# mutiann/few-shot-transformer-tts

Measured on AMD Instinct MI355X. Metric: padded mel-frames/sec, full training step (fwd+loss+bwd+allreduce+Adam), higher is better.
Workload: dtype bf16; 1 GPU; LJSpeech-shaped (BASELINE configs[1]) packed batch per GPU: B=14 S=114 T=582, default hparams (83.5M params), dropout on, single speaker/language; global_batch=14, seq_len=582, parallelism=dp1

## Files before the change

### few-shot-transformer-tts_amd/csrc/attention32.hip

```cpp
#include "b2s_common.h"
#include "attention.h"

namespace {

typedef __attribute__((ext_vector_type(16))) float f32x16_t;
typedef __attribute__((ext_vector_type(4))) uint32_t u32x4_t;
typedef __attribute__((address_space(3))) bf16x4_t* lds_b64_ptr;

typedef __attribute__((address_space(1))) void* gptr_t;
typedef __attribute__((address_space(3))) void* lptr_t;
__device__ inline f32x16_t mma32(bf16x8_t a, bf16x8_t b, f32x16_t c) { return __builtin_amdgcn_mfma_f32_32x32x16_bf16(a, b, c, 0, 0, 0); }
__device__ inline float half_max(float v) {
    const uint32_t u = __float_as_uint(v);
    const auto r = __builtin_amdgcn_permlane32_swap(u, u, false, false);
    return fmaxf(__uint_as_float(r[0]), __uint_as_float(r[1]));
}
__device__ inline float half_sum(float v) {
    const uint32_t u = __float_as_uint(v);
    const auto r = __builtin_amdgcn_permlane32_swap(u, u, false, false);
    return __uint_as_float(r[0]) + __uint_as_float(r[1]);
}
__device__ inline float fast_exp2(float x) { return __builtin_amdgcn_exp2f(x); }
__device__ inline float vmax3(float a, float b, float c) { float d; asm("v_max3_f32 %0, %1, %2, %3" : "=v"(d) : "v"(a), "v"(b), "v"(c)); return d; }
constexpr float A32_LOG2E = 1.4426950408889634f, A32_LN2 = 0.6931471805599453f;
constexpr float A32_LAZY = 8.f;

template <int DH> __device__ inline int swz(int row) { return DH == 64 ? ((((row >> 1) & 1) << 2) | ((row >> 2) & 3)) : ((row >> 2) & 3); }

template <int DH, int NW> struct Dma {
    static constexpr int CPR = DH / 8, NI = CPR / NW;
    static_assert(CPR % NW == 0, "tile must split evenly over the waves");
    int row[NI], cb[NI];
    const char* base; uint32_t ldb; int last;
    __device__ inline void init(const bf16_t* b, long ld_, int nrows_, int wave, int lane) {
        base = reinterpret_cast<const char*>(b); ldb = (uint32_t)ld_ * 2u; last = nrows_ - 1;
#pragma unroll
        for (int i = 0; i < NI; ++i) {
            const int p = (wave * NI + i) * 64 + lane, r = p / CPR, c = (p - r * CPR) ^ swz<DH>(r);
            row[i] = r; cb[i] = c * 16;
        }
    }
    __device__ inline void issue(bf16_t* tile, int row0, int wave) const {
#pragma unroll
        for (int i = 0; i < NI; ++i) {
            const uint32_t voff = (uint32_t)min(row0 + row[i], last) * ldb + (uint32_t)cb[i];
            __builtin_amdgcn_global_load_lds((gptr_t)(base + voff), (lptr_t)(tile + (wave * NI + i) * 512), 16, 0, 0);
        }
    }
};
__device__ inline void cfence() { asm volatile("" ::: "memory"); }
__device__ inline void wait_vm0() { asm volatile("s_waitcnt vmcnt(0)" ::: "memory"); }
template <int DH> __device__ inline bf16x8_t frag_a(const bf16_t* tile, int row, int ks, int hi) {
    return *reinterpret_cast<const bf16x8_t*>(tile + row * DH + (((ks * 2 + hi) ^ swz<DH>(row)) * 8));
}
template <int DH> __device__ inline bf16x8_t frag_t(const bf16_t* tile, int rb, int d0, int lane) {
    const int li = lane & 15, g = lane >> 4;
    const int row = rb + (g >> 1) * 4 + (li >> 2), col = d0 + (g & 1) * 16 + (li & 3) * 4;
    const bf16_t* p0 = tile + row * DH + (((col >> 3) ^ swz<DH>(row)) * 8) + (col & 7);
    const bf16_t* p1 = tile + (row + 8) * DH + (((col >> 3) ^ swz<DH>(row + 8)) * 8) + (col & 7);
    const bf16x4_t lo = __builtin_amdgcn_ds_read_tr16_b64_v4i16((lds_b64_ptr)p0);
    const bf16x4_t hh = __builtin_amdgcn_ds_read_tr16_b64_v4i16((lds_b64_ptr)p1);
    bf16x8_t r;
    r[0] = lo[0]; r[1] = lo[1]; r[2] = lo[2]; r[3] = lo[3]; r[4] = hh[0]; r[5] = hh[1]; r[6] = hh[2]; r[7] = hh[3];
    return r;
}
template <int S8> __device__ inline bf16x8_t pack8(const f32x16_t& v) {
    const u32x4_t u = {f2bf2(v[S8 * 8 + 0], v[S8 * 8 + 1]), f2bf2(v[S8 * 8 + 2], v[S8 * 8 + 3]), f2bf2(v[S8 * 8 + 4], v[S8 * 8 + 5]),
                       f2bf2(v[S8 * 8 + 6], v[S8 * 8 + 7])};
    return __builtin_bit_cast(bf16x8_t, u);
}
__device__ inline bf16x8_t frag_own(const bf16_t* base, long ld, int row, int ks, int hi) {
    return *reinterpret_cast<const bf16x8_t*>(base + (long)row * ld + ks * 16 + hi * 8);
}
__device__ inline float frag_dot(bf16x8_t x, bf16x8_t y) {
    float s = 0.f;
#pragma unroll
    for (int e = 0; e < 8; ++e) s += bf2f((bf16_t)x[e]) * bf2f((bf16_t)y[e]);
    return s;
}
__device__ inline int crow(int r, int hi) { return (r & 3) + 8 * (r >> 2) + 4 * hi; }

__device__ inline void a32_block(int& rank, int& z) {
    const int nx = gridDim.x, Z = gridDim.y, orig = blockIdx.y * nx + blockIdx.x;
    if ((Z & 7) == 0) {
        const int zc = Z >> 3, x = orig & 7, i = orig >> 3;
        rank = i / zc; z = x * zc + (i - rank * zc);
    } else {
        const int nwg = nx * Z, xcd = orig & 7, q = nwg >> 3, r = nwg & 7;
        const int wg = (xcd < r ? xcd * (q + 1) : r * (q + 1) + (xcd - r) * q) + (orig >> 3);
        z = wg / nx; rank = wg - z * nx;
    }
}
template <int DH>
__device__ inline void store_own(bf16_t* dst, const f32x16_t (&acc)[DH / 32], float mul, int hi) {
#pragma unroll
    for (int dt = 0; dt < DH / 32; ++dt)
#pragma unroll
        for (int g4 = 0; g4 < 4; ++g4) {
            uint2 u;
            u.x = f2bf2(acc[dt][g4 * 4 + 0] * mul, acc[dt][g4 * 4 + 1] * mul);
            u.y = f2bf2(acc[dt][g4 * 4 + 2] * mul, acc[dt][g4 * 4 + 3] * mul);
            *reinterpret_cast<uint2*>(dst + dt * 32 + g4 * 8 + hi * 4) = u;
        }
}
template <int DH> __device__ inline void zero_own(bf16_t* dst, int hi) {
#pragma unroll
    for (int dt = 0; dt < DH / 32; ++dt)
#pragma unroll
        for (int g4 = 0; g4 < 4; ++g4) *reinterpret_cast<uint2*>(dst + dt * 32 + g4 * 8 + hi * 4) = make_uint2(0, 0);
}
constexpr uint32_t GOLD = 0x9E3779B1u;


template <int DH>
__device__ inline void first2(f32x16_t (&s)[2], const bf16_t* tile, const bf16x8_t (&own)[DH / 16], int l31, int hi) {
#pragma unroll
    for (int t = 0; t < 2; ++t) {
#pragma unroll
        for (int r = 0; r < 16; ++r) s[t][r] = 0.f;
#pragma unroll
        for (int ks = 0; ks < DH / 16; ++ks) s[t] = mma32(frag_a<DH>(tile, t * 32 + l31, ks, hi), own[ks], s[t]);
    }
}
template <int DH>
__device__ inline void first1(f32x16_t& s, const bf16_t* tile, int t, const bf16x8_t (&own)[DH / 16], int l31, int hi) {
#pragma unroll
    for (int r = 0; r < 16; ++r) s[r] = 0.f;
#pragma unroll
    for (int ks = 0; ks < DH / 16; ++ks) s = mma32(frag_a<DH>(tile, t * 32 + l31, ks, hi), own[ks], s);
}
template <int DH>
__device__ inline void second1(f32x16_t (&acc)[DH / 32], const bf16_t* tile, int t, const f32x16_t& w, int lane) {
    const bf16x8_t p0 = pack8<0>(w), p1 = pack8<1>(w);
#pragma unroll
    for (int dt = 0; dt < DH / 32; ++dt) {
        acc[dt] = mma32(frag_t<DH>(tile, t * 32, dt * 32, lane), p0, acc[dt]);
        acc[dt] = mma32(frag_t<DH>(tile, t * 32 + 16, dt * 32, lane), p1, acc[dt]);
    }
}
__device__ inline void quad_words(uint32_t (&wd)[16], uint32_t xrow, int k0) {
    const uint32_t xt = xrow + (uint32_t)(k0 >> 2) * GOLD;
#pragma unroll
    for (int t = 0; t < 2; ++t)
#pragma unroll
        for (int g4 = 0; g4 < 4; ++g4) {
            const uint32_t x = xt + (uint32_t)(t * 8 + g4 * 2) * GOLD, y = x ^ (x >> 16);
            wd[t * 8 + g4 * 2] = y * B2S_WC0; wd[t * 8 + g4 * 2 + 1] = y * B2S_WC1;
        }
}
__device__ inline uint32_t keep_mask16(uint32_t w, uint32_t tsm1, uint32_t fifteen) {
    uint32_t d, m;
    asm("v_pk_sub_i16 %0, %1, %2 clamp" : "=v"(d) : "v"(tsm1), "v"(w));
    asm("v_pk_ashrrev_i16 %0, %1, %2" : "=v"(m) : "v"(fifteen), "v"(d));
    return m;
}
template <int S8> __device__ inline bf16x8_t pack8_drop(const f32x16_t& v, const uint32_t* wd, uint32_t tsm1, uint32_t fifteen) {
    const u32x4_t u = {f2bf2(v[S8 * 8 + 0], v[S8 * 8 + 1]) & keep_mask16(wd[S8 * 4 + 0], tsm1, fifteen), f2bf2(v[S8 * 8 + 2], v[S8 * 8 + 3]) & keep_mask16(wd[S8 * 4 + 1], tsm1, fifteen),
                       f2bf2(v[S8 * 8 + 4], v[S8 * 8 + 5]) & keep_mask16(wd[S8 * 4 + 2], tsm1, fifteen), f2bf2(v[S8 * 8 + 6], v[S8 * 8 + 7]) & keep_mask16(wd[S8 * 4 + 3], tsm1, fifteen)};
    return __builtin_bit_cast(bf16x8_t, u);
}
template <int DH>
__device__ inline void second1p(f32x16_t (&acc)[DH / 32], const bf16_t* tile, int t, bf16x8_t p0, bf16x8_t p1, int lane) {
#pragma unroll
    for (int dt = 0; dt < DH / 32; ++dt) {
        acc[dt] = mma32(frag_t<DH>(tile, t * 32, dt * 32, lane), p0, acc[dt]);
        acc[dt] = mma32(frag_t<DH>(tile, t * 32 + 16, dt * 32, lane), p1, acc[dt]);
    }
}

template <int DH, int NW, bool DROP>
__global__ __launch_bounds__(NW * 64, 2) void attn32_fwd_kernel(AttnArgs a) {
    constexpr int NKS = DH / 16, NDT = DH / 32, TILE = 64 * DH, QB = NW * 32;
    __shared__ __attribute__((aligned(16))) bf16_t sK[2 * TILE];
    __shared__ __attribute__((aligned(16))) bf16_t sV[2 * TILE];
    const int tid = threadIdx.x, lane = tid & 63, wave = tid >> 6, l31 = lane & 31, hi = lane >> 5;
    int blk, z;
    a32_block(blk, z);
    blk = gridDim.x - 1 - blk;
    const int b = z / a.H, h = z - b * a.H;
    const int qrow0 = a.qoff ? a.qoff[b] : b * a.Lq, Lq = a.qoff ? a.qoff[b + 1] - qrow0 : a.Lq;
    const int krow0 = a.koff ? a.koff[b] : b * a.Lk, Lk = a.koff ? a.koff[b + 1] - krow0 : a.Lk;
    const int qb0 = blk * QB, qw0 = qb0 + wave * 32, q = qw0 + l31, qc = min(q, Lq - 1);
    const int qlive = a.qskip ? min(a.qskip[b], Lq) : Lq;
    const bool wlive = (qw0 & ~63) < qlive && qw0 < Lq;
    bf16_t* out = reinterpret_cast<bf16_t*>(a.out) + ((long)qrow0 + qc) * a.ldo + h * DH;
    if (!wlive && q < Lq) {
        zero_own<DH>(out, hi);
        if (hi == 0 && a.lse) a.lse[(long)z * a.Lq + q] = 0.f;
    }
    if (qb0 >= qlive) return;
    const bf16_t* Q = reinterpret_cast<const bf16_t*>(a.q) + (long)qrow0 * a.ldq + h * DH;
    const bf16_t* K = reinterpret_cast<const bf16_t*>(a.k) + (long)krow0 * a.ldk + h * DH;
    const bf16_t* V = reinterpret_cast<const bf16_t*>(a.v) + (long)krow0 * a.ldv + h * DH;
    const bool causal = a.mask_mode & 2;
    int kend = Lk;
    if (a.mask_mode & 1) kend = min(kend, a.klen[b]);
    int ktiles = (kend + 63) / 64;
    if (causal) {
        int qlast = min(qb0 + QB - 1, Lq - 1);
        if (a.qskip) qlast = min(qlast, ((qlive + 63) & ~63) - 1);
        ktiles = min(ktiles, qlast / 64 + 1);
    }
    const int wkt = !wlive ? 0 : (causal ? min(ktiles, min(qw0 + 31, Lq - 1) / 64 + 1) : ktiles);
    Dma<DH, NW> dmk, dmv;
    dmk.init(K, a.ldk, Lk, wave, lane); dmv.init(V, a.ldv, Lk, wave, lane);
    if (ktiles > 0) { dmk.issue(sK, 0, wave); dmv.issue(sV, 0, wave); }
    if (ktiles > 1) dmk.issue(sK + TILE, 64, wave);
    bf16x8_t qf[NKS];
#pragma unroll
    for (int ks = 0; ks < NKS; ++ks) qf[ks] = frag_own(Q, a.ldq, qc, ks, hi);

    f32x16_t o[NDT];
#pragma unroll
    for (int dt = 0; dt < NDT; ++dt)
#pragma unroll
        for (int r = 0; r < 16; ++r) o[dt][r] = 0.f;
    float m = -INFINITY, l = 0.f;
    const float sl2 = a.scale * A32_LOG2E;
    const uint32_t xrow = b2s_wseed(a.drop, (uint32_t)((long)z * a.Lq + qc)) + (uint32_t)hi * GOLD;
    const uint32_t tsm1 = ((uint32_t)(b2s_wthresh(a.drop) - 1) & 0xffffu) * 0x10001u, fifteen = 0x000f000fu;
    f32x16_t s0[2], s1[2];
    uint32_t wd[16];
    wait_vm0();
    __syncthreads();
    if (wkt > 0) {
        first2<DH>(s0, sK, qf, l31, hi);
        if (DROP) quad_words(wd, xrow, 0);
    }
    __syncthreads();
    auto iter = [&](const int kt, f32x16_t (&sc)[2], f32x16_t (&sn)[2]) {
        const int k0 = kt * 64, cur = kt & 1;
        if (kt + 2 < ktiles) dmk.issue(sK + cur * TILE, k0 + 128, wave);
        if (kt + 1 < ktiles) dmv.issue(sV + (cur ^ 1) * TILE, k0 + 64, wave);
        if (kt < wkt) {
            const bool interior = k0 + 64 <= kend && (!causal || k0 + 63 <= qw0);
            if (!interior) {
#pragma unroll
                for (int t = 0; t < 2; ++t)
#pragma unroll
                    for (int r = 0; r < 16; ++r) {
                        const int key = k0 + t * 32 + crow(r, hi);
                        sc[t][r] = (key < kend && (!causal || key <= q)) ? sc[t][r] : -INFINITY;
                    }
            }
            float mx = sc[0][0];
#pragma unroll
            for (int r = 0; r < 16; ++r) mx = vmax3(mx, sc[0][r], sc[1][r]);
            mx = half_max(mx) * sl2;
            const bool grow = mx > m + A32_LAZY;
            if (__any(grow)) {
                const float mn = grow ? mx : m;
                const float alpha = mn == m ? 1.f : fast_exp2(m - mn);
                m = mn; l *= alpha;
#pragma unroll
                for (int dt = 0; dt < NDT; ++dt)
#pragma unroll
                    for (int r = 0; r < 16; ++r) o[dt][r] *= alpha;
            }
            const float mref = m == -INFINITY ? 0.f : m;
            first2<DH>(sn, sK + (cur ^ 1) * TILE, qf, l31, hi);
#pragma unroll
            for (int t = 0; t < 2; ++t)
#pragma unroll
                for (int r = 0; r < 16; ++r) {
                    const float p = fast_exp2(fmaf(sc[t][r], sl2, -mref));
                    l += p;
                    sc[t][r] = p;
                }
            if (DROP) {
                second1p<DH>(o, sV + cur * TILE, 0, pack8_drop<0>(sc[0], wd, tsm1, fifteen), pack8_drop<1>(sc[0], wd, tsm1, fifteen), lane);
                second1p<DH>(o, sV + cur * TILE, 1, pack8_drop<0>(sc[1], wd + 8, tsm1, fifteen), pack8_drop<1>(sc[1], wd + 8, tsm1, fifteen), lane);
            } else {
                second1<DH>(o, sV + cur * TILE, 0, sc[0], lane);
                second1<DH>(o, sV + cur * TILE, 1, sc[1], lane);
            }
            if (DROP) quad_words(wd, xrow, k0 + 64);
        }
        wait_vm0();
        __syncthreads();
    };
    for (int kt = 0; kt < ktiles; kt += 2) {
        iter(kt, s0, s1);
        if (kt + 1 < ktiles) iter(kt + 1, s1, s0);
    }
    l = half_sum(l);
    if (wlive && q < Lq) {
        const float inv = 1.f / l;
        store_own<DH>(out, o, inv * a.drop.scale, hi);
        if (hi == 0 && a.lse) a.lse[(long)z * a.Lq + q] = (m + __log2f(l)) * A32_LN2;
    }
}

template <int DH, int NW, bool DROP>
__global__ __launch_bounds__(NW * 64, 2) void attn32_dq_kernel(AttnArgs a) {
    constexpr int NKS = DH / 16, NDT = DH / 32, TILE = 64 * DH, QB = NW * 32;
    __shared__ __attribute__((aligned(16))) bf16_t sK[2 * TILE];
    __shared__ __attribute__((aligned(16))) bf16_t sV[2 * TILE];
    const int tid = threadIdx.x, lane = tid & 63, wave = tid >> 6, l31 = lane & 31, hi = lane >> 5;
    int blk, z;
    a32_block(blk, z);
    blk = gridDim.x - 1 - blk;
    const int b = z / a.H, h = z - b * a.H;
    const int qrow0 = a.qoff ? a.qoff[b] : b * a.Lq, Lq = a.qoff ? a.qoff[b + 1] - qrow0 : a.Lq;
    const int krow0 = a.koff ? a.koff[b] : b * a.Lk, Lk = a.koff ? a.koff[b + 1] - krow0 : a.Lk;
    const int qb0 = blk * QB, qw0 = qb0 + wave * 32, q = qw0 + l31, qc = min(q, Lq - 1);
    const int qlive = a.qskip ? min(a.qskip[b], Lq) : Lq;
    const bool wlive = (qw0 & ~63) < qlive && qw0 < Lq;
    bf16_t* dqo = reinterpret_cast<bf16_t*>(a.dq) + ((long)qrow0 + qc) * a.lddq + h * DH;
    if (!wlive && q < Lq) {
        zero_own<DH>(dqo, hi);
        if (hi == 0) a.dsum[(long)z * a.Lq + q] = 0.f;
    }
    if (qb0 >= qlive) return;
    const bf16_t* Q = reinterpret_cast<const bf16_t*>(a.q) + (long)qrow0 * a.ldq + h * DH;
    const bf16_t* K = reinterpret_cast<const bf16_t*>(a.k) + (long)krow0 * a.ldk + h * DH;
    const bf16_t* V = reinterpret_cast<const bf16_t*>(a.v) + (long)krow0 * a.ldv + h * DH;
    const bf16_t* dO = reinterpret_cast<const bf16_t*>(a.dout) + (long)qrow0 * a.ldo + h * DH;
    const bf16_t* O = reinterpret_cast<const bf16_t*>(a.oref) + (long)qrow0 * a.ldo + h * DH;
    const bool causal = a.mask_mode & 2;
    int kend = Lk;
    if (a.mask_mode & 1) kend = min(kend, a.klen[b]);
    int ktiles = (kend + 63) / 64;
    if (causal) {
        int qlast = min(qb0 + QB - 1, Lq - 1);
        if (a.qskip) qlast = min(qlast, ((qlive + 63) & ~63) - 1);
        ktiles = min(ktiles, qlast / 64 + 1);
    }
    const int wkt = !wlive ? 0 : (causal ? min(ktiles, min(qw0 + 31, Lq - 1) / 64 + 1) : ktiles);
    Dma<DH, NW> dmk, dmv;
    dmk.init(K, a.ldk, Lk, wave, lane); dmv.init(V, a.ldv, Lk, wave, lane);
    if (ktiles > 0) { dmk.issue(sK, 0, wave); dmv.issue(sV, 0, wave); }
    bf16x8_t qf[NKS], dof[NKS];
    float Dq = 0.f;
#pragma unroll
    for (int ks = 0; ks < NKS; ++ks) {
        qf[ks] = frag_own(Q, a.ldq, qc, ks, hi); dof[ks] = frag_own(dO, a.ldo, qc, ks, hi);
        Dq += frag_dot(frag_own(O, a.ldo, qc, ks, hi), dof[ks]);
    }
    Dq = half_sum(Dq);
    if (wlive && hi == 0 && q < Lq) a.dsum[(long)z * a.Lq + q] = Dq;
    f32x16_t dq[NDT];
#pragma unroll
    for (int dt = 0; dt < NDT; ++dt)
#pragma unroll
        for (int r = 0; r < 16; ++r) dq[dt][r] = 0.f;
    const float sl2 = a.scale * A32_LOG2E, lse2 = a.lse[(long)z * a.Lq + qc] * A32_LOG2E;
    const uint32_t xrow = b2s_wseed(a.drop, (uint32_t)((long)z * a.Lq + qc)) + (uint32_t)hi * GOLD;
    const int ts32 = (int)((uint32_t)b2s_wthresh(a.drop) << 16);
    const float dscale = a.drop.scale;
    wait_vm0();
    __syncthreads();
    for (int kt = 0; kt < ktiles; ++kt) {
        const int k0 = kt * 64, cur = kt & 1;
        const bf16_t* tK = sK + cur * TILE;
        const bf16_t* tV = sV + cur * TILE;
        if (kt + 1 < ktiles) { dmk.issue(sK + (cur ^ 1) * TILE, k0 + 64, wave); dmv.issue(sV + (cur ^ 1) * TILE, k0 + 64, wave); }
        if (kt < wkt) {
            const bool interior = k0 + 64 <= kend && (!causal || k0 + 63 <= qw0);
            f32x16_t s[2], dp[2];
            first2<DH>(s, tK, qf, l31, hi);
            first2<DH>(dp, tV, dof, l31, hi);
            if (!interior) {
#pragma unroll
                for (int t = 0; t < 2; ++t)
#pragma unroll
                    for (int r = 0; r < 16; ++r) {
                        const int key = k0 + t * 32 + crow(r, hi);
                        s[t][r] = (key < kend && (!causal || key <= q)) ? s[t][r] : -INFINITY;
                    }
            }
            uint32_t wd[16];
            if (DROP) quad_words(wd, xrow, k0);
#pragma unroll
            for (int t = 0; t < 2; ++t) {
#pragma unroll
                for (int r = 0; r < 16; ++r) s[t][r] = fast_exp2(fmaf(s[t][r], sl2, -lse2));
                if (DROP) {
#pragma unroll
                    for (int pr = 0; pr < 8; ++pr) {
                        const uint32_t w = wd[t * 8 + pr];
                        dp[t][2 * pr] = (int)(w << 16) >= ts32 ? dp[t][2 * pr] * dscale : 0.f;
                        dp[t][2 * pr + 1] = (int)w >= ts32 ? dp[t][2 * pr + 1] * dscale : 0.f;
                    }
                }
#pragma unroll
                for (int r = 0; r < 16; ++r) s[t][r] = s[t][r] * (dp[t][r] - Dq);
                second1<DH>(dq, tK, t, s[t], lane);
            }
        }
        wait_vm0();
        __syncthreads();
    }
    if (wlive && q < Lq) store_own<DH>(dqo, dq, a.scale, hi);
}

template <int DH, int NW, bool DROP>
__global__ __launch_bounds__(NW * 64, 2) void attn32_dkv_kernel(AttnArgs a) {
    constexpr int NKS = DH / 16, NDT = DH / 32, TILE = 64 * DH, KB = NW * 32;
    __shared__ __attribute__((aligned(16))) bf16_t sQ[2 * TILE];
    __shared__ __attribute__((aligned(16))) bf16_t sO[2 * TILE];
    __shared__ __attribute__((aligned(16))) float sL[2 * 64], sD[2 * 64];
    __shared__ __attribute__((aligned(16))) uint32_t sS[2 * 64];
    const int tid = threadIdx.x, lane = tid & 63, wave = tid >> 6, l31 = lane & 31, hi = lane >> 5;
    int blk, z;
    a32_block(blk, z);
    const int b = z / a.H, h = z - b * a.H;
    const int qrow0 = a.qoff ? a.qoff[b] : b * a.Lq, Lq = a.qoff ? a.qoff[b + 1] - qrow0 : a.Lq;
    const int krow0 = a.koff ? a.koff[b] : b * a.Lk, Lk = a.koff ? a.koff[b + 1] - krow0 : a.Lk;
    const int kb0 = blk * KB, kw0 = kb0 + wave * 32, key = kw0 + l31, kc = min(key, Lk - 1);
    int kend = Lk;
    if (a.mask_mode & 1) kend = min(kend, a.klen[b]);
    bf16_t* dko = reinterpret_cast<bf16_t*>(a.dk) + ((long)krow0 + kc) * a.lddk + h * DH;
    bf16_t* dvo = reinterpret_cast<bf16_t*>(a.dv) + ((long)krow0 + kc) * a.lddv + h * DH;
    const bool wlive = kw0 < kend;
    if (!wlive && key < Lk) { zero_own<DH>(dko, hi); zero_own<DH>(dvo, hi); }
    if (kb0 >= kend) return;
    const bool causal = a.mask_mode & 2;
    const bf16_t* Q = reinterpret_cast<const bf16_t*>(a.q) + (long)qrow0 * a.ldq + h * DH;
    const bf16_t* K = reinterpret_cast<const bf16_t*>(a.k) + (long)krow0 * a.ldk + h * DH;
    const bf16_t* V = reinterpret_cast<const bf16_t*>(a.v) + (long)krow0 * a.ldv + h * DH;
    const bf16_t* dO = reinterpret_cast<const bf16_t*>(a.dout) + (long)qrow0 * a.ldo + h * DH;
    int qtiles = (Lq + 63) / 64;
    if (a.qskip) qtiles = min(qtiles, (a.qskip[b] + 63) / 64);
    const int qt0 = causal ? kb0 / 64 : 0;
    const int wqt0 = !wlive ? qtiles : (causal ? kw0 / 64 : 0);
    Dma<DH, NW> dmq, dmo;
    dmq.init(Q, a.ldq, Lq, wave, lane); dmo.init(dO, a.ldo, Lq, wave, lane);
    float r_l = 0.f, r_d = 0.f;
    uint32_t r_s = 0;
    if (qt0 < qtiles) {
        dmq.issue(sQ + (qt0 & 1) * TILE, qt0 * 64, wave); dmo.issue(sO + (qt0 & 1) * TILE, qt0 * 64, wave);
        if (tid < 64) {
            const int qq = min(qt0 * 64 + tid, Lq - 1);
            sL[(qt0 & 1) * 64 + tid] = a.lse[(long)z * a.Lq + qq] * A32_LOG2E; sD[(qt0 & 1) * 64 + tid] = a.dsum[(long)z * a.Lq + qq];
            if (DROP) sS[(qt0 & 1) * 64 + tid] = b2s_wseed(a.drop, (uint32_t)((long)z * a.Lq + qq));
        }
    }
    bf16x8_t kf[NKS], vf[NKS];
#pragma unroll
    for (int ks = 0; ks < NKS; ++ks) { kf[ks] = frag_own(K, a.ldk, kc, ks, hi); vf[ks] = frag_own(V, a.ldv, kc, ks, hi); }
    const bool key_ok = key < kend;
    f32x16_t dk[NDT], dv[NDT];
#pragma unroll
    for (int dt = 0; dt < NDT; ++dt)
#pragma unroll
        for (int r = 0; r < 16; ++r) { dk[dt][r] = 0.f; dv[dt][r] = 0.f; }
    const float sl2 = a.scale * A32_LOG2E, dscale = a.drop.scale;
    const uint32_t xk = (uint32_t)(kc >> 2) * GOLD, wck = (kc & 2) ? B2S_WC1 : B2S_WC0, hsh = (kc & 1) ? 0u : 16u;
    const int ts32 = (int)((uint32_t)b2s_wthresh(a.drop) << 16);
    wait_vm0();
    __syncthreads();
    for (int qt = qt0; qt < qtiles; ++qt) {
        const int q0 = qt * 64, cur = qt & 1;
        const bf16_t* tQ = sQ + cur * TILE;
        const bf16_t* tO = sO + cur * TILE;
        const float* tL = sL + cur * 64;
        const float* tD = sD + cur * 64;
        const uint32_t* tS = sS + cur * 64;
        if (qt + 1 < qtiles) {
            dmq.issue(sQ + (cur ^ 1) * TILE, q0 + 64, wave); dmo.issue(sO + (cur ^ 1) * TILE, q0 + 64, wave);
            if (tid < 64) {
                const int qq = min(q0 + 64 + tid, Lq - 1);
                r_l = a.lse[(long)z * a.Lq + qq] * A32_LOG2E; r_d = a.dsum[(long)z * a.Lq + qq];
                if (DROP) r_s = b2s_wseed(a.drop, (uint32_t)((long)z * a.Lq + qq));
            }
        }
        if (qt >= wqt0) {
            const bool interior = kw0 + 32 <= kend && q0 + 64 <= Lq && (!causal || kw0 + 31 <= q0);
#pragma unroll
            for (int t = 0; t < 2; ++t) {
                f32x16_t s, dp;
                first1<DH>(s, tQ, t, kf, l31, hi);
                cfence();
                first1<DH>(dp, tO, t, vf, l31, hi);
                cfence();
                if (!interior) {
#pragma unroll
                    for (int r = 0; r < 16; ++r) {
                        const int qq = q0 + t * 32 + crow(r, hi);
                        s[r] = (key_ok && qq < Lq && (!causal || key <= qq)) ? s[r] : -INFINITY;
                    }
                }
#pragma unroll
                for (int g4 = 0; g4 < 4; ++g4) {
                    const f32x4_t lq = *reinterpret_cast<const f32x4_t*>(tL + t * 32 + g4 * 8 + hi * 4);
#pragma unroll
                    for (int j = 0; j < 4; ++j) s[g4 * 4 + j] = fast_exp2(fmaf(s[g4 * 4 + j], sl2, -lq[j]));
                }
#pragma unroll
                for (int g4 = 0; g4 < 4; ++g4) {
                    const f32x4_t d4 = *reinterpret_cast<const f32x4_t*>(tD + t * 32 + g4 * 8 + hi * 4);
                    u32x4_t sd4 = {0, 0, 0, 0};
                    if (DROP) sd4 = *reinterpret_cast<const u32x4_t*>(tS + t * 32 + g4 * 8 + hi * 4);
#pragma unroll
                    for (int j = 0; j < 4; ++j) {
                        const int r = g4 * 4 + j;
                        bool keep = true;
                        if (DROP) {
                            const uint32_t x = sd4[j] + xk;
                            keep = (int)(((x ^ (x >> 16)) * wck) << hsh) >= ts32;
                        }
                        const float d = keep ? dp[r] * dscale : 0.f;
                        dp[r] = s[r] * (d - d4[j]);
                        s[r] = keep ? s[r] : 0.f;
                    }
                }
                cfence();
                second1<DH>(dv, tO, t, s, lane);
                cfence();
                second1<DH>(dk, tQ, t, dp, lane);
                cfence();
            }
        }
        if (qt + 1 < qtiles && tid < 64) { sL[(cur ^ 1) * 64 + tid] = r_l; sD[(cur ^ 1) * 64 + tid] = r_d; if (DROP) sS[(cur ^ 1) * 64 + tid] = r_s; }
        wait_vm0();
        __syncthreads();
    }
    if (wlive && key < Lk) { store_own<DH>(dko, dk, a.scale, hi); store_own<DH>(dvo, dv, dscale, hi); }
}

template <int DH, bool DROP>
int launch32(const AttnArgs& a, int which, hipStream_t st) {
    constexpr int NW = 4;
    if (which == 0) {
        hipLaunchKernelGGL((attn32_fwd_kernel<DH, NW, DROP>), dim3(cdiv(a.Lq, NW * 32), a.B * a.H), dim3(NW * 64), 0, st, a);
    } else if (which == 1) {
        hipLaunchKernelGGL((attn32_dq_kernel<DH, NW, DROP>), dim3(cdiv(a.Lq, NW * 32), a.B * a.H), dim3(NW * 64), 0, st, a);
    } else {
        hipLaunchKernelGGL((attn32_dkv_kernel<DH, NW, DROP>), dim3(cdiv(a.Lk, NW * 32), a.B * a.H), dim3(NW * 64), 0, st, a);
    }
    B2S_LAUNCH_CHECK();
    return 0;
}
template <int DH>
int launch32_dh(const AttnArgs& a, int which, hipStream_t st) {
    return (a.drop.thresh >> 16) != 0 ? launch32<DH, true>(a, which, st) : launch32<DH, false>(a, which, st);
}
}

bool b2s_flash32_supported(int dh) { return dh == 32 || dh == 64 || dh == 96; }
int b2s_flash32_launch(const AttnArgs& a, int dh, int which, hipStream_t st) {
    B2S_CHECK(!a.ga_rows, "the 32x32 attention kernels do not carry the guided-attention term (it belongs to the encoder-decoder attention: attention.hip)");
    switch (dh) {
        case 32: return launch32_dh<32>(a, which, st);
        case 64: return launch32_dh<64>(a, which, st);
        case 96: return launch32_dh<96>(a, which, st);
    }
    return b2s_fail(__FILE__, __LINE__, "bf16 attention supports head sizes 32/64/96 (got %d)", dh);
}
```

Measured before the change: 1.228 million mel-frames/s.

## Split long causal attention blocks across helper workgroups with merge via workspace

For causal self-attention, the key-tile (or query-tile, in dK/dV) range of the longest blocks is split between the original workgroup and an extra helper workgroup. The two halves are combined through a global workspace and an atomic counter: online-softmax rescaling in the forward pass, and summation for dQ and dK/dV. Launch order is permuted so the longest work slots start first, which shortens the tail caused by causal imbalance. The cost is extra launched blocks, workspace traffic, atomics, and a persistent device buffer allocated on first use.

```diff
diff --git a/few-shot-transformer-tts_amd/csrc/attention32.hip b/few-shot-transformer-tts_amd/csrc/attention32.hip
--- a/few-shot-transformer-tts_amd/csrc/attention32.hip
+++ b/few-shot-transformer-tts_amd/csrc/attention32.hip
@@ -1,5 +1,7 @@
 #include "b2s_common.h"
 #include "attention.h"
+#include <algorithm>
+#include <mutex>
 
 namespace {
 
@@ -111,6 +113,62 @@
 }
 constexpr uint32_t GOLD = 0x9E3779B1u;
 
+constexpr int A32_SPLIT_MIN = 7;
+constexpr int A32_MAXSLOT = 16;
+struct A32Split {
+    float* ws = nullptr;
+    int* cnt = nullptr;
+    int nblk = 0, nhelp = 0, first = 0;
+    int smin = 0;
+    unsigned long long order = 0;
+};
+__device__ inline void a32_slot(const A32Split& sp, int rank, int rank_blk, int& blk, int& helper) {
+    blk = rank_blk; helper = 0;
+    if (sp.nhelp) {
+        const int s = (int)(sp.order >> (rank * 4)) & 15;
+        helper = s >= sp.nblk;
+        blk = helper ? sp.first + s - sp.nblk : s;
+    }
+}
+__device__ inline bool a32_has_helper(const A32Split& sp, int blk) { return sp.nhelp && blk >= sp.first && blk < sp.first + sp.nhelp; }
+template <int NV, int NX>
+__device__ inline bool split_publish(const A32Split& sp, int slot, int helper, int tid, const f32x16_t* acc, const float* x, volatile int* flag) {
+    constexpr int PER = (NV * 16 + NX) * 256;
+    float* mine = sp.ws + ((size_t)slot * 2 + helper) * PER;
+#pragma unroll
+    for (int v = 0; v < NV; ++v)
+#pragma unroll
+        for (int g4 = 0; g4 < 4; ++g4)
+            *reinterpret_cast<f32x4_t*>(mine + ((v * 4 + g4) * 256 + tid) * 4) = f32x4_t{acc[v][g4 * 4], acc[v][g4 * 4 + 1], acc[v][g4 * 4 + 2], acc[v][g4 * 4 + 3]};
+#pragma unroll
+    for (int i = 0; i < NX; ++i) mine[(NV * 16 + i) * 256 + tid] = x[i];
+    wait_vm0();
+    __syncthreads();
+    if (tid == 0) {
+        __builtin_amdgcn_fence(__ATOMIC_RELEASE, "agent");
+        wait_vm0();
+        const int old = __hip_atomic_fetch_add(sp.cnt + slot, 1, __ATOMIC_RELAXED, __HIP_MEMORY_SCOPE_AGENT);
+        if (old) {
+            __builtin_amdgcn_fence(__ATOMIC_ACQUIRE, "agent");
+            wait_vm0();
+            __hip_atomic_store(sp.cnt + slot, 0, __ATOMIC_RELAXED, __HIP_MEMORY_SCOPE_AGENT);
+        }
+        *flag = old;
+    }
+    __syncthreads();
+    return *flag != 0;
+}
+template <int NV, int NX>
+__device__ inline f32x4_t split_other(const A32Split& sp, int slot, int helper, int tid, int v, int g4) {
+    constexpr int PER = (NV * 16 + NX) * 256;
+    return *reinterpret_cast<const f32x4_t*>(sp.ws + ((size_t)slot * 2 + (helper ^ 1)) * PER + ((v * 4 + g4) * 256 + tid) * 4);
+}
+template <int NV, int NX>
+__device__ inline float split_other_x(const A32Split& sp, int slot, int helper, int tid, int i) {
+    constexpr int PER = (NV * 16 + NX) * 256;
+    return sp.ws[((size_t)slot * 2 + (helper ^ 1)) * PER + (NV * 16 + i) * 256 + tid];
+}
+
 
 template <int DH>
 __device__ inline void first2(f32x16_t (&s)[2], const bf16_t* tile, const bf16x8_t (&own)[DH / 16], int l31, int hi) {
@@ -169,14 +227,14 @@
 }
 
 template <int DH, int NW, bool DROP>
-__global__ __launch_bounds__(NW * 64, 2) void attn32_fwd_kernel(AttnArgs a) {
+__global__ __launch_bounds__(NW * 64, 2) void attn32_fwd_kernel(AttnArgs a, A32Split sp) {
     constexpr int NKS = DH / 16, NDT = DH / 32, TILE = 64 * DH, QB = NW * 32;
     __shared__ __attribute__((aligned(16))) bf16_t sK[2 * TILE];
     __shared__ __attribute__((aligned(16))) bf16_t sV[2 * TILE];
     const int tid = threadIdx.x, lane = tid & 63, wave = tid >> 6, l31 = lane & 31, hi = lane >> 5;
-    int blk, z;
-    a32_block(blk, z);
-    blk = gridDim.x - 1 - blk;
+    int rank, z, blk, helper;
+    a32_block(rank, z);
+    a32_slot(sp, rank, gridDim.x - 1 - rank, blk, helper);
     const int b = z / a.H, h = z - b * a.H;
     const int qrow0 = a.qoff ? a.qoff[b] : b * a.Lq, Lq = a.qoff ? a.qoff[b + 1] - qrow0 : a.Lq;
     const int krow0 = a.koff ? a.koff[b] : b * a.Lk, Lk = a.koff ? a.koff[b + 1] - krow0 : a.Lk;
@@ -184,7 +242,7 @@
     const int qlive = a.qskip ? min(a.qskip[b], Lq) : Lq;
     const bool wlive = (qw0 & ~63) < qlive && qw0 < Lq;
     bf16_t* out = reinterpret_cast<bf16_t*>(a.out) + ((long)qrow0 + qc) * a.ldo + h * DH;
-    if (!wlive && q < Lq) {
+    if (!wlive && q < Lq && !helper) {
         zero_own<DH>(out, hi);
         if (hi == 0 && a.lse) a.lse[(long)z * a.Lq + q] = 0.f;
     }
@@ -201,11 +259,15 @@
         if (a.qskip) qlast = min(qlast, ((qlive + 63) & ~63) - 1);
         ktiles = min(ktiles, qlast / 64 + 1);
     }
+    const bool split = causal && a32_has_helper(sp, blk) && ktiles >= sp.smin;
+    if (helper && !split) return;
+    int kt0 = 0;
+    if (split) { if (helper) kt0 = ktiles >> 1; else ktiles >>= 1; }
     const int wkt = !wlive ? 0 : (causal ? min(ktiles, min(qw0 + 31, Lq - 1) / 64 + 1) : ktiles);
     Dma<DH, NW> dmk, dmv;
     dmk.init(K, a.ldk, Lk, wave, lane); dmv.init(V, a.ldv, Lk, wave, lane);
-    if (ktiles > 0) { dmk.issue(sK, 0, wave); dmv.issue(sV, 0, wave); }
-    if (ktiles > 1) dmk.issue(sK + TILE, 64, wave);
+    if (ktiles > kt0) { dmk.issue(sK, kt0 * 64, wave); dmv.issue(sV, kt0 * 64, wave); }
+    if (ktiles > kt0 + 1) dmk.issue(sK + TILE, kt0 * 64 + 64, wave);
     bf16x8_t qf[NKS];
 #pragma unroll
     for (int ks = 0; ks < NKS; ++ks) qf[ks] = frag_own(Q, a.ldq, qc, ks, hi);
@@ -223,13 +285,13 @@
     uint32_t wd[16];
     wait_vm0();
     __syncthreads();
-    if (wkt > 0) {
+    if (wkt > kt0) {
         first2<DH>(s0, sK, qf, l31, hi);
-        if (DROP) quad_words(wd, xrow, 0);
+        if (DROP) quad_words(wd, xrow, kt0 * 64);
     }
     __syncthreads();
     auto iter = [&](const int kt, f32x16_t (&sc)[2], f32x16_t (&sn)[2]) {
-        const int k0 = kt * 64, cur = kt & 1;
+        const int k0 = kt * 64, cur = (kt - kt0) & 1;
         if (kt + 2 < ktiles) dmk.issue(sK + cur * TILE, k0 + 128, wave);
         if (kt + 1 < ktiles) dmv.issue(sV + (cur ^ 1) * TILE, k0 + 64, wave);
         if (kt < wkt) {
@@ -279,9 +341,30 @@
         wait_vm0();
         __syncthreads();
     };
-    for (int kt = 0; kt < ktiles; kt += 2) {
+    for (int kt = kt0; kt < ktiles; kt += 2) {
         iter(kt, s0, s1);
         if (kt + 1 < ktiles) iter(kt + 1, s1, s0);
+    }
+    if (split) {
+        const int slot = z * sp.nhelp + blk - sp.first;
+        const float x[2] = {m, l};
+        if (!split_publish<NDT, 2>(sp, slot, helper, tid, o, x, reinterpret_cast<volatile int*>(sK))) return;
+        const float mo = split_other_x<NDT, 2>(sp, slot, helper, tid, 0), lo = split_other_x<NDT, 2>(sp, slot, helper, tid, 1);
+        const float m_lo = helper ? mo : m, m_hi = helper ? m : mo, l_lo = helper ? lo : l, l_hi = helper ? l : lo;
+        const float mn = fmaxf(m_lo, m_hi);
+        const float a_lo = m_lo == mn ? 1.f : fast_exp2(m_lo - mn), a_hi = m_hi == mn ? 1.f : fast_exp2(m_hi - mn);
+        m = mn; l = __fmaf_rn(l_lo, a_lo, __fmul_rn(l_hi, a_hi));
+#pragma unroll
+        for (int dt = 0; dt < NDT; ++dt)
+#pragma unroll
+            for (int g4 = 0; g4 < 4; ++g4) {
+                const f32x4_t oo = split_other<NDT, 2>(sp, slot, helper, tid, dt, g4);
+#pragma unroll
+                for (int j = 0; j < 4; ++j) {
+                    const float own = o[dt][g4 * 4 + j], o_lo = helper ? oo[j] : own, o_hi = helper ? own : oo[j];
+                    o[dt][g4 * 4 + j] = __fmaf_rn(o_lo, a_lo, __fmul_rn(o_hi, a_hi));
+                }
+            }
     }
     l = half_sum(l);
     if (wlive && q < Lq) {
@@ -292,14 +375,14 @@
 }
 
 template <int DH, int NW, bool DROP>
-__global__ __launch_bounds__(NW * 64, 2) void attn32_dq_kernel(AttnArgs a) {
+__global__ __launch_bounds__(NW * 64, 2) void attn32_dq_kernel(AttnArgs a, A32Split sp) {
     constexpr int NKS = DH / 16, NDT = DH / 32, TILE = 64 * DH, QB = NW * 32;
     __shared__ __attribute__((aligned(16))) bf16_t sK[2 * TILE];
     __shared__ __attribute__((aligned(16))) bf16_t sV[2 * TILE];
     const int tid = threadIdx.x, lane = tid & 63, wave = tid >> 6, l31 = lane & 31, hi = lane >> 5;
-    int blk, z;
-    a32_block(blk, z);
-    blk = gridDim.x - 1 - blk;
+    int rank, z, blk, helper;
+    a32_block(rank, z);
+    a32_slot(sp, rank, gridDim.x - 1 - rank, blk, helper);
     const int b = z / a.H, h = z - b * a.H;
     const int qrow0 = a.qoff ? a.qoff[b] : b * a.Lq, Lq = a.qoff ? a.qoff[b + 1] - qrow0 : a.Lq;
     const int krow0 = a.koff ? a.koff[b] : b * a.Lk, Lk = a.koff ? a.koff[b + 1] - krow0 : a.Lk;
@@ -307,7 +390,7 @@
     const int qlive = a.qskip ? min(a.qskip[b], Lq) : Lq;
     const bool wlive = (qw0 & ~63) < qlive && qw0 < Lq;
     bf16_t* dqo = reinterpret_cast<bf16_t*>(a.dq) + ((long)qrow0 + qc) * a.lddq + h * DH;
-    if (!wlive && q < Lq) {
+    if (!wlive && q < Lq && !helper) {
         zero_own<DH>(dqo, hi);
         if (hi == 0) a.dsum[(long)z * a.Lq + q] = 0.f;
     }
@@ -326,10 +409,14 @@
         if (a.qskip) qlast = min(qlast, ((qlive + 63) & ~63) - 1);
         ktiles = min(ktiles, qlast / 64 + 1);
     }
+    const bool split = causal && a32_has_helper(sp, blk) && ktiles >= sp.smin;
+    if (helper && !split) return;
+    int kt0 = 0;
+    if (split) { if (helper) kt0 = ktiles >> 1; else ktiles >>= 1; }
     const int wkt = !wlive ? 0 : (causal ? min(ktiles, min(qw0 + 31, Lq - 1) / 64 + 1) : ktiles);
     Dma<DH, NW> dmk, dmv;
     dmk.init(K, a.ldk, Lk, wave, lane); dmv.init(V, a.ldv, Lk, wave, lane);
-    if (ktiles > 0) { dmk.issue(sK, 0, wave); dmv.issue(sV, 0, wave); }
+    if (ktiles > kt0) { dmk.issue(sK, kt0 * 64, wave); dmv.issue(sV, kt0 * 64, wave); }
     bf16x8_t qf[NKS], dof[NKS];
     float Dq = 0.f;
 #pragma unroll
@@ -338,7 +425,7 @@
         Dq += frag_dot(frag_own(O, a.ldo, qc, ks, hi), dof[ks]);
     }
     Dq = half_sum(Dq);
-    if (wlive && hi == 0 && q < Lq) a.dsum[(long)z * a.Lq + q] = Dq;
+    if (wlive && hi == 0 && q < Lq && !helper) a.dsum[(long)z * a.Lq + q] = Dq;
     f32x16_t dq[NDT];
 #pragma unroll
     for (int dt = 0; dt < NDT; ++dt)
@@ -350,8 +437,8 @@
     const float dscale = a.drop.scale;
     wait_vm0();
     __syncthreads();
-    for (int kt = 0; kt < ktiles; ++kt) {
-        const int k0 = kt * 64, cur = kt & 1;
+    for (int kt = kt0; kt < ktiles; ++kt) {
+        const int k0 = kt * 64, cur = (kt - kt0) & 1;
         const bf16_t* tK = sK + cur * TILE;
         const bf16_t* tV = sV + cur * TILE;
         if (kt + 1 < ktiles) { dmk.issue(sK + (cur ^ 1) * TILE, k0 + 64, wave); dmv.issue(sV + (cur ^ 1) * TILE, k0 + 64, wave); }
@@ -391,19 +478,32 @@
         wait_vm0();
         __syncthreads();
     }
+    if (split) {
+        const int slot = z * sp.nhelp + blk - sp.first;
+        if (!split_publish<NDT, 0>(sp, slot, helper, tid, dq, nullptr, reinterpret_cast<volatile int*>(sK))) return;
+#pragma unroll
+        for (int dt = 0; dt < NDT; ++dt)
+#pragma unroll
+            for (int g4 = 0; g4 < 4; ++g4) {
+                const f32x4_t oo = split_other<NDT, 0>(sp, slot, helper, tid, dt, g4);
+#pragma unroll
+                for (int j = 0; j < 4; ++j) dq[dt][g4 * 4 + j] += oo[j];
+            }
+    }
     if (wlive && q < Lq) store_own<DH>(dqo, dq, a.scale, hi);
 }
 
 template <int DH, int NW, bool DROP>
-__global__ __launch_bounds__(NW * 64, 2) void attn32_dkv_kernel(AttnArgs a) {
+__global__ __launch_bounds__(NW * 64, 2) void attn32_dkv_kernel(AttnArgs a, A32Split sp) {
     constexpr int NKS = DH / 16, NDT = DH / 32, TILE = 64 * DH, KB = NW * 32;
     __shared__ __attribute__((aligned(16))) bf16_t sQ[2 * TILE];
     __shared__ __attribute__((aligned(16))) bf16_t sO[2 * TILE];
     __shared__ __attribute__((aligned(16))) float sL[2 * 64], sD[2 * 64];
     __shared__ __attribute__((aligned(16))) uint32_t sS[2 * 64];
     const int tid = threadIdx.x, lane = tid & 63, wave = tid >> 6, l31 = lane & 31, hi = lane >> 5;
-    int blk, z;
-    a32_block(blk, z);
+    int rank, z, blk, helper;
+    a32_block(rank, z);
+    a32_slot(sp, rank, rank, blk, helper);
     const int b = z / a.H, h = z - b * a.H;
     const int qrow0 = a.qoff ? a.qoff[b] : b * a.Lq, Lq = a.qoff ? a.qoff[b + 1] - qrow0 : a.Lq;
     const int krow0 = a.koff ? a.koff[b] : b * a.Lk, Lk = a.koff ? a.koff[b + 1] - krow0 : a.Lk;
@@ -413,7 +513,7 @@
     bf16_t* dko = reinterpret_cast<bf16_t*>(a.dk) + ((long)krow0 + kc) * a.lddk + h * DH;
     bf16_t* dvo = reinterpret_cast<bf16_t*>(a.dv) + ((long)krow0 + kc) * a.lddv + h * DH;
     const bool wlive = kw0 < kend;
-    if (!wlive && key < Lk) { zero_own<DH>(dko, hi); zero_own<DH>(dvo, hi); }
+    if (!wlive && key < Lk && !helper) { zero_own<DH>(dko, hi); zero_own<DH>(dvo, hi); }
     if (kb0 >= kend) return;
     const bool causal = a.mask_mode & 2;
     const bf16_t* Q = reinterpret_cast<const bf16_t*>(a.q) + (long)qrow0 * a.ldq + h * DH;
@@ -422,7 +522,10 @@
     const bf16_t* dO = reinterpret_cast<const bf16_t*>(a.dout) + (long)qrow0 * a.ldo + h * DH;
     int qtiles = (Lq + 63) / 64;
     if (a.qskip) qtiles = min(qtiles, (a.qskip[b] + 63) / 64);
-    const int qt0 = causal ? kb0 / 64 : 0;
+    int qt0 = causal ? kb0 / 64 : 0;
+    const bool split = causal && a32_has_helper(sp, blk) && qtiles - qt0 >= sp.smin;
+    if (helper && !split) return;
+    if (split) { const int n = qtiles - qt0; if (helper) qt0 += n >> 1; else qtiles = qt0 + (n >> 1); }
     const int wqt0 = !wlive ? qtiles : (causal ? kw0 / 64 : 0);
     Dma<DH, NW> dmq, dmo;
     dmq.init(Q, a.ldq, Lq, wave, lane); dmo.init(dO, a.ldo, Lq, wave, lane);
@@ -516,18 +619,85 @@
         wait_vm0();
         __syncthreads();
     }
+    if (split) {
+        const int slot = z * sp.nhelp + blk - sp.first;
+        f32x16_t both[2 * NDT];
+#pragma unroll
+        for (int dt = 0; dt < NDT; ++dt) { both[dt] = dk[dt]; both[NDT + dt] = dv[dt]; }
+        if (!split_publish<2 * NDT, 0>(sp, slot, helper, tid, both, nullptr, reinterpret_cast<volatile int*>(sQ))) return;
+#pragma unroll
+        for (int dt = 0; dt < NDT; ++dt)
+#pragma unroll
+            for (int g4 = 0; g4 < 4; ++g4) {
+                const f32x4_t ok = split_other<2 * NDT, 0>(sp, slot, helper, tid, dt, g4), ov = split_other<2 * NDT, 0>(sp, slot, helper, tid, NDT + dt, g4);
+#pragma unroll
+                for (int j = 0; j < 4; ++j) { dk[dt][g4 * 4 + j] += ok[j]; dv[dt][g4 * 4 + j] += ov[j]; }
+            }
+    }
     if (wlive && key < Lk) { store_own<DH>(dko, dk, a.scale, hi); store_own<DH>(dvo, dv, dscale, hi); }
 }
 
+#ifdef B2S_LAB
+static const int g_split_min = getenv("B2S_LAB_ATTN_SPLIT") ? atoi(getenv("B2S_LAB_ATTN_SPLIT")) : A32_SPLIT_MIN;
+static const int g_split_which = getenv("B2S_LAB_ATTN_SPLIT_WHICH") ? atoi(getenv("B2S_LAB_ATTN_SPLIT_WHICH")) : 7;
+#else
+constexpr int g_split_min = A32_SPLIT_MIN;
+constexpr int g_split_which = 7;
+#endif
+bool split_buffers(int which, size_t nslot, size_t slot_floats, A32Split& sp) {
+    constexpr int MAXDEV = 16;
+    struct Buf { char* p = nullptr; size_t nslot = 0, bytes = 0; };
+    static Buf pool[MAXDEV][3];
+    static std::mutex mu;
+    int dev = 0;
+    if (hipGetDevice(&dev) != hipSuccess || dev < 0 || dev >= MAXDEV) { (void)hipGetLastError(); return false; }
+    const size_t cbytes = (nslot * sizeof(int) + 255) & ~(size_t)255, bytes = cbytes + nslot * slot_floats * sizeof(float);
+    std::lock_guard<std::mutex> lock(mu);
+    Buf& b = pool[dev][which];
+    if (b.nslot < nslot || b.bytes < bytes) {
+        void* p = nullptr;
+        if (hipMalloc(&p, bytes) != hipSuccess || hipMemset(p, 0xff, bytes) != hipSuccess || hipMemset(p, 0, cbytes) != hipSuccess) {
+            (void)hipGetLastError();
+            return false;
+        }
+        b.p = (char*)p; b.nslot = nslot; b.bytes = bytes;
+    }
+    sp.cnt = reinterpret_cast<int*>(b.p);
+    sp.ws = reinterpret_cast<float*>(b.p + ((b.nslot * sizeof(int) + 255) & ~(size_t)255));
+    return true;
+}
+template <int DH>
+void plan_split(A32Split& sp, const AttnArgs& a, int which) {
+    const int smin = g_split_min;
+    if (smin < 2 || !((g_split_which >> which) & 1) || !(a.mask_mode & 2) || a.Lq != a.Lk) return;
+    const int T = cdiv(a.Lq, 64), nblk = cdiv(a.Lq, 128);
+    if (T < smin) return;
+    const int first = which == 2 ? 0 : (smin + 1) / 2 - 1, nhelp = which == 2 ? (T - smin) / 2 + 1 : nblk - first;
+    if (nhelp <= 0 || nblk + nhelp > A32_MAXSLOT) return;
+    int len[A32_MAXSLOT], slot[A32_MAXSLOT];
+    for (int s = 0; s < nblk + nhelp; ++s) {
+        const int i = s < nblk ? s : first + s - nblk, n = which == 2 ? T - 2 * i : std::min(T, 2 * i + 2);
+        const bool sh = i >= first && i < first + nhelp;
+        len[s] = !sh ? n : (s < nblk ? n / 2 : n - n / 2);
+        slot[s] = s;
+    }
+    std::stable_sort(slot, slot + nblk + nhelp, [&](int x, int y) { return len[x] > len[y]; });
+    constexpr size_t slot_floats = 2 * (size_t)256 * ((DH / 32) * 16 * 2 + 2);
+    if (!split_buffers(which, (size_t)a.B * a.H * nhelp, slot_floats, sp)) return;
+    sp.nblk = nblk; sp.nhelp = nhelp; sp.first = first; sp.smin = smin; sp.order = 0;
+    for (int r = 0; r < nblk + nhelp; ++r) sp.order |= (unsigned long long)slot[r] << (4 * r);
+}
 template <int DH, bool DROP>
 int launch32(const AttnArgs& a, int which, hipStream_t st) {
     constexpr int NW = 4;
+    A32Split sp;
+    plan_split<DH>(sp, a, which);
     if (which == 0) {
-        hipLaunchKernelGGL((attn32_fwd_kernel<DH, NW, DROP>), dim3(cdiv(a.Lq, NW * 32), a.B * a.H), dim3(NW * 64), 0, st, a);
+        hipLaunchKernelGGL((attn32_fwd_kernel<DH, NW, DROP>), dim3(cdiv(a.Lq, NW * 32) + sp.nhelp, a.B * a.H), dim3(NW * 64), 0, st, a, sp);
     } else if (which == 1) {
-        hipLaunchKernelGGL((attn32_dq_kernel<DH, NW, DROP>), dim3(cdiv(a.Lq, NW * 32), a.B * a.H), dim3(NW * 64), 0, st, a);
+        hipLaunchKernelGGL((attn32_dq_kernel<DH, NW, DROP>), dim3(cdiv(a.Lq, NW * 32) + sp.nhelp, a.B * a.H), dim3(NW * 64), 0, st, a, sp);
     } else {
-        hipLaunchKernelGGL((attn32_dkv_kernel<DH, NW, DROP>), dim3(cdiv(a.Lk, NW * 32), a.B * a.H), dim3(NW * 64), 0, st, a);
+        hipLaunchKernelGGL((attn32_dkv_kernel<DH, NW, DROP>), dim3(cdiv(a.Lk, NW * 32) + sp.nhelp, a.B * a.H), dim3(NW * 64), 0, st, a, sp);
     }
     B2S_LAUNCH_CHECK();
     return 0;
```

Measured after the change: 1.144 million mel-frames/s. -6.8%, worse.
